# Nature40/pyradiotracking

Hardware: AMD Instinct MI355X
Metric: IQ MSamples/s analysed (STFT + detect + records), detected-signal parity vs CPU (higher is better)
Workload: dtype f32

## Files before the change

pyradiotracking_amd/csrc/rt_analyze.hip:

```cpp
#include <hip/hip_runtime.h>

#include <algorithm>
#include <cmath>
#include <cstdio>
#include <cstdlib>
#include <cstring>
#include <limits>
#include <new>
#include <string>
#include <type_traits>
#include <vector>

#include "rt_kernels.h"
#include "rt_general.h"
#include "rt_f64.h"
#include "rt_f64_sparse.h"
#include "rt_f64_rescue.h"
#include "rt_cells.h"
#include "rt_present.h"
#include "rt_chain.h"
#include "rt_record_iq.h"
#include "rt_record_stft.h"
#include "rt_record_stft_hop.h"
#include "rt_record_estimates.h"
// ... 219 lines not shown
struct InputStatsState {
    bool on = false;
    int max_chunks = 0;
    InputStatsSlot slot[kSlots];
};

}

struct rt_handle {
    rt_config cfg{};
    int R3 = 1, N = 256, LG = 16, GPW = 16;
    bool wcos = false;
    int big = 0;
    int QS = 0;
    int K = 1;
    int stride = 1;
    int L = 32;
    int max_seg = 0;
    std::vector<float> h_thr_s;
    int max_chunks = 0;
    bool two_level = false;
    int max_blocks = 0;
    hipStream_t s_scan = nullptr;
    bool own_scan_stream = false;
    hipStream_t s_detect = nullptr;
    std::string err;

    bool general = false;
    int log2n = 8;
    cf *d_twg = nullptr;
    bool bluestein = false;
    int gen_m = 0;
    cf *d_cwin = nullptr;
    cf *d_bfilt = nullptr;
    int n_cu = 256;
    uint32_t *d_work = nullptr;
    float *d_window = nullptr;
    float *d_window_t = nullptr;
    cf *d_tw1 = nullptr, *d_tw2 = nullptr;
    float *d_tail[kTails] = {nullptr, nullptr, nullptr};
    float *d_spec = nullptr;
    float *d_spec_part = nullptr;
    void *d_iq_stage[kSlots] = {nullptr, nullptr};
    size_t iq_stage_bytes[kSlots] = {0, 0};
    int64_t pool_want = 0;
    int64_t pool_max = 0;
    Slot slot[kSlots];

    int hot_cap = 8192, rec_cap = 1024, cand_cap = 32;
    bool group_detect = false;
    bool group_light = true;
    bool group_forced = false;
    size_t lds_large = 0, lds_small = 0, lds_dense = 0;

    bool lin = false;
    int32_t *d_sub_first = nullptr;
    std::vector<int32_t> h_sub_first;
    int32_t *h_sub_list = nullptr;
    int n_sub = 0;
    uint64_t sub_epoch = 0;
    float lin_c[3] = {0.f, 0.f, 0.f};

    AutoPolicy ap;
    int minsum_slot = -1;
    int run_cells = 1;
    uint64_t n_calls = 0;
    uint64_t test_enqueues = 0;
    int test_fail_lane = -1, test_fail_nth = 0;
    int tail_mode = 0;
    StreamLedger ledger;
    LedgerCall lc_saved;
    float *d_thr_s = nullptr, *d_cal_s = nullptr;
    StreamSettings *d_set_s = nullptr;
    std::vector<StreamSettings> h_set_s;

    rt_call_info info{};
    bool timing = false;

    std::vector<rt_handle *> kids;
    std::vector<int> kid_base;

    int rm_slot = -1;
    bool cells_full = false;
    int64_t cells_want = 0;

    size_t chunk_min_bytes = 0;
    const Slot *launch_mask = nullptr;
    std::vector<float> h_cal_s;

    F64State *f64 = nullptr;
    RecordIq *riq = nullptr;
    int iq_margin = -1;
    InputStatsState *ist = nullptr;
    std::vector<float> h_window;
};

namespace {

#define RT_HIP(h, expr)                                                                       \
    do {                                                                                      \
        hipError_t e_ = (expr);                                                               \
        if (e_ != hipSuccess) {                                                               \
            (h)->err = std::string(#expr) + ": " + hipGetErrorString(e_);                     \
            return RT_E_HIP;                                                                  \
        }                                                                                     \
    } while (0)

#ifdef RT_DIAG
extern "C" char **environ;
void warn_unknown_switches() {
    static bool done = false;
    if (done) return;
    done = true;
    static const char *const known[] = {"RT_EXP_ONE_LEVEL", "RT_EXP_TAIL", "RT_EXP_STREAMS", "RT_EXP_TAIL_PRIO", "RT_TEST_FAIL_LANE", "RT_STAMPS_DUMP"};
    for (char **e = environ; e && *e; ++e) {
        if (std::strncmp(*e, "RT_EXP_", 7) != 0 && std::strncmp(*e, "RT_TEST_", 8) != 0) continue;
        const char *eq = std::strchr(*e, '=');
        const std::string name(*e, eq ? (size_t)(eq - *e) : std::strlen(*e));
        bool ok = false;
        for (const char *k : known) ok = ok || name == k;
        if (!ok) std::fprintf(stderr, "librt_analyze_diag: environment variable %s is set but this build reads no such switch (known: RT_EXP_ONE_LEVEL, RT_EXP_TAIL, RT_EXP_STREAMS, RT_EXP_TAIL_PRIO, RT_TEST_FAIL_LANE, RT_STAMPS_DUMP)\n", name.c_str());
    }
}
#endif

#define RT_DEVICE_COPY(CHECK, dst, src, bytes)                     \
    do {                                                           \
        CHECK(hipMalloc(&dst, bytes));                             \
        CHECK(hipMemcpy(dst, src, bytes, hipMemcpyHostToDevice));  \
    } while (0)
#define RT_DEVICE_ZEROS(CHECK, dst, bytes) \
    do {                                   \
        CHECK(hipMalloc(&dst, bytes));     \
        CHECK(hipMemset(dst, 0, bytes));   \
    } while (0)

int fail_create(int code, const std::string &msg) {
    g_create_error = msg;
    return code;
}

size_t rec_lds_bytes(int rec_cap) { return (size_t)std::min(rec_cap, kDenseLdsRecords) * (8 + 8 + sizeof(rt_record)) + 16; }

void launch_detect_dense(rt_handle *h, int grid, hipStream_t st, const DetectArgs &a);

#define RT_SCAN_KERNEL(R3_, QS_) (stft_scan<R3_, MODEF, FMT == kFmtU8, LIN, QS_>)
#define RT_WG_KERNEL(B_, W_) (stft_wg<B_, MODEF, FMT == kFmtU8, W_>)
template <int MODE, int FMT, bool LIN>
void launch_stft_lin(rt_handle *h, const StftParams &p, int items, hipStream_t st) {
    constexpr int MODEF = MODE | (FMT == kFmtI16 ? kModeI16 : FMT == kFmtI8 ? kModeI8 : 0);
    if (h->big) {
        if constexpr (MODE <= 2) {
            if (h->big == 256) {
                if (h->wcos) hipLaunchKernelGGL(RT_WG_KERNEL(256, true), dim3(items), dim3(256), wg_lds_bytes(256), st, p);
                else hipLaunchKernelGGL(RT_WG_KERNEL(256, false), dim3(items), dim3(256), wg_lds_bytes(256), st, p);
            } else {
                if (h->wcos) hipLaunchKernelGGL(RT_WG_KERNEL(512, true), dim3(items), dim3(512), wg_lds_bytes(512), st, p);
                else hipLaunchKernelGGL(RT_WG_KERNEL(512, false), dim3(items), dim3(512), wg_lds_bytes(512), st, p);
            }
        }
        return;
    }
    if (scan_wave64(h->R3)) {
        const int wgs = std::min((items + kW64Waves - 1) / kW64Waves, h->n_cu);
        hipLaunchKernelGGL((stft_scan64<MODEF, FMT == kFmtU8, LIN>), dim3(wgs), dim3(kW64Block), 0, st, p);
        return;
    }
    const int blk = scan_block(h->R3);
    const int per_cu = scan_dma(h->R3, FMT, h->QS) ? 2 : std::min(((h->R3 <= RT_WG4_MAX_R3 || (FMT == kFmtU8 && h->R3 == 1)) ? 4 : 3) * (kBlock / blk), blk == 64 ? 12 : 4);
    const bool persist = scan_persistent(h->R3, MODE);
    const int blocks = persist ? std::min(items, h->n_cu * per_cu) : items;
    switch (h->QS ? -h->QS : h->R3) {
        case -8: hipLaunchKernelGGL(RT_SCAN_KERNEL(1, 8), dim3(blocks), dim3(blk), 0, st, p); break;
        case -4: hipLaunchKernelGGL(RT_SCAN_KERNEL(1, 4), dim3(blocks), dim3(blk), 0, st, p); break;
        case -2: hipLaunchKernelGGL(RT_SCAN_KERNEL(1, 2), dim3(blocks), dim3(blk), 0, st, p); break;
        case 1: hipLaunchKernelGGL(RT_SCAN_KERNEL(1, 0), dim3(blocks), dim3(blk), 0, st, p); break;
        case 2: hipLaunchKernelGGL(RT_SCAN_KERNEL(2, 0), dim3(blocks), dim3(blk), 0, st, p); break;
        case 4: hipLaunchKernelGGL(RT_SCAN_KERNEL(4, 0), dim3(blocks), dim3(blk), 0, st, p); break;
        case 8: hipLaunchKernelGGL(RT_SCAN_KERNEL(8, 0), dim3(blocks), dim3(blk), 0, st, p); break;
#if !RT_WAVE64_4096
        default: hipLaunchKernelGGL(RT_SCAN_KERNEL(16, 0), dim3(blocks), dim3(blk), 0, st, p); break;
#else
        default: break;
#endif
    }
}
#undef RT_SCAN_KERNEL
#undef RT_WG_KERNEL

template <int MODE, int FMT = kFmtC64>
void launch_stft(rt_handle *h, const StftParams &p, int blocks, hipStream_t st) {
    constexpr bool U8 = (FMT == kFmtU8);
    const Slot *const mk = (MODE != 3 && !p.stream_list) ? h->launch_mask : nullptr;
    if (mk) {
        const int S = h->cfg.n_streams;
        const int n_present = mk->lc.pc.n_present;
        if (n_present == 0) return;
        StftParams q = p;
        if (h->lin && !U8) {
            if (mk->n_lin_present > 0) {
                q.sub_first = nullptr;
                q.stream_list = mk->d_mask + (size_t)kMaskLinList * S;
                q.n_streams = mk->n_lin_present;
                q.spec_by_stream = 1;
                launch_stft_lin<MODE, FMT, (MODE != 3 && !U8)>(h, q, q.n_streams * p.blocks_per_stream, st);
            }
            if (mk->n_sub_present == 0) return;
            q = p;
            q.stream_list = mk->d_mask + (size_t)kMaskSubList * S;
            q.n_streams = mk->n_sub_present;
        } else {
            q.stream_list = mk->d_mask + (size_t)kMaskList * S;
            q.n_streams = n_present;
        }
        q.sub_first = nullptr;
        q.dc_flag = h->lin && !U8 ? nullptr : p.dc_flag;
        q.spec_by_stream = 1;
        launch_stft_lin<MODE, FMT, false>(h, q, q.n_streams * p.blocks_per_stream, st);
        return;
    }
    if (h->lin && MODE != 3 && !U8) {
        if (p.stream_list || h->n_sub == 0 || !p.sub_first) {
            StftParams q = p;
            if (p.stream_list) q.sub_first = nullptr;
            launch_stft_lin<MODE, FMT, (MODE != 3 && !U8)>(h, q, blocks, st);
        } else {
            launch_stft_lin<MODE, FMT, (MODE != 3 && !U8)>(h, p, blocks, st);
            StftParams q = p;
            q.sub_first = nullptr;
            q.dc_flag = nullptr;
            q.spec_by_stream = 1;
            q.stream_list = h->h_sub_list;
            q.n_streams = h->n_sub;
            launch_stft_lin<MODE, FMT, false>(h, q, h->n_sub * p.blocks_per_stream, st);
        }
    } else {
        launch_stft_lin<MODE, FMT, false>(h, p, blocks, st);
    }
}

void launch_general(rt_handle *h, const void *iq, int64_t stream_stride, int n_seg, float *spec, float *tail, int fmt, const int32_t *absent = nullptr) {
    if (h->bluestein) {
        BluesteinParams b{};
        b.absent = absent;
        b.iq = iq;
        b.stream_stride = stream_stride;
        b.n_streams = h->cfg.n_streams;
        b.n_seg = n_seg;
        b.nperseg = h->N;
        b.m = h->gen_m;
        b.log2m = h->log2n;
        b.tail_cols = h->K;
        b.cwin = h->d_cwin;
        b.bfilt = h->d_bfilt;
        b.tw = h->d_twg;
        b.spec = spec;
        b.tail = tail;
        const int blocks = h->cfg.n_streams * n_seg;
        const size_t lds = (size_t)h->gen_m * sizeof(cf);
#define RT_BLU(U_, B_)                                                                                                            \
    do {                                                                                                                          \
        if (fmt == kFmtU8) hipLaunchKernelGGL((stft_bluestein<kFmtU8, U_, B_>), dim3(blocks), dim3(B_), lds, h->s_scan, b);        \
        else if (fmt == kFmtI16) hipLaunchKernelGGL((stft_bluestein<kFmtI16, U_, B_>), dim3(blocks), dim3(B_), lds, h->s_scan, b); \
        else if (fmt == kFmtI8) hipLaunchKernelGGL((stft_bluestein<kFmtI8, U_, B_>), dim3(blocks), dim3(B_), lds, h->s_scan, b);   \
        else hipLaunchKernelGGL((stft_bluestein<kFmtC64, U_, B_>), dim3(blocks), dim3(B_), lds, h->s_scan, b);                     \
    } while (0)
        if (h->gen_m >= 16384) RT_BLU(4, 1024);
        else if (h->gen_m >= 8192) RT_BLU(4, 512);
        else if (h->gen_m >= 4096) RT_BLU(2, 512);
        else if (h->gen_m >= 2048) RT_BLU(2, 256);
        else RT_BLU(1, 256);
#undef RT_BLU
        return;
    }
    GeneralParams g{};
    g.absent = absent;
    g.iq = iq;
    g.stream_stride = stream_stride;
    g.n_streams = h->cfg.n_streams;
    g.n_seg = n_seg;
    g.nperseg = h->N;
    g.log2n = h->log2n;
    g.segs_per_block = std::min(64, std::max(1, 1024 / h->N));
    g.tail_cols = h->K;
    g.window = h->d_window;
    g.tw = h->d_twg;
    g.spec = spec;
    g.tail = tail;
    const int blocks = h->cfg.n_streams * ((n_seg + g.segs_per_block - 1) / g.segs_per_block);
    const size_t lds = (size_t)g.segs_per_block * h->N * sizeof(cf);
    if (fmt == kFmtU8) hipLaunchKernelGGL((stft_general<kFmtU8>), dim3(blocks), dim3(kGeneralBlock), lds, h->s_scan, g);
    else if (fmt == kFmtI16) hipLaunchKernelGGL((stft_general<kFmtI16>), dim3(blocks), dim3(kGeneralBlock), lds, h->s_scan, g);
    else if (fmt == kFmtI8) hipLaunchKernelGGL((stft_general<kFmtI8>), dim3(blocks), dim3(kGeneralBlock), lds, h->s_scan, g);
    else hipLaunchKernelGGL((stft_general<kFmtC64>), dim3(blocks), dim3(kGeneralBlock), lds, h->s_scan, g);
}

long long min_run_cells(const rt_handle *h) { return rt::min_run_cells(h->N, h->cfg.sample_rate, h->cfg.min_duration_s); }

int choose_chunk(const rt_config &cfg, const ScanFamily &fam, int n_streams, int n_seg) {
    return rt::choose_chunk(cfg.nperseg, fam.R3, fam.QS, scan_block(fam.R3), cfg.sample_rate, cfg.min_duration_s, cfg.segs_per_chunk, n_streams, n_seg);
}


StftParams make_stft_params(rt_handle *h, Slot &sl, const void *iq, int64_t stream_stride, int n_seg, int tail_write) {
    StftParams p{};
    p.iq = iq;
    p.stream_stride = stream_stride;
    p.n_streams = h->cfg.n_streams;
    p.n_seg = n_seg;
    p.segs_per_chunk = h->L;
    p.chunks = (n_seg + h->L - 1) / h->L;
// ... 4020 lines not shown
```

pyradiotracking_amd/csrc/rt_diag.h:

```cpp
#ifndef RT_DIAG_H
#define RT_DIAG_H

#ifdef RT_DIAG
#include <cstdlib>
#define RT_DIAG_ENV(name) std::getenv(name)
#else
#define RT_DIAG_ENV(name) (static_cast<const char *>(nullptr))
#if defined(RT_STAMPS) || defined(RT_ABLATE) || defined(RT_DETECT_ABLATE) || defined(RT_W64_ABL) || defined(RT_WG_ABL) || defined(RT_EXP_WG_HALF) || defined(RT_EXP_DMA1024) || defined(RT_EXP_WG_NOFENCE) || defined(RT_EXP_NOBAR0) || defined(RT_EXP_NOBAR1) || \
    defined(RT_EXP_ALIAS) || defined(RT_EXP_NOWIN) || defined(RT_EXP_PRIO) || defined(RT_ONE_WAVE_MAX_R3) || defined(RT_NO_PERSIST) ||                    \
    defined(RT_WG4_MAX_R3) || defined(RT_PK_R3_MASK) || defined(RT_BELOW_MAX_R3) || defined(RT_WAVE64_4096) || defined(RT_W64_PK) ||                       \
    defined(RT_W64_PREFETCH) || defined(RT_W64_Q2AHEAD) || defined(RT_EXP6) || defined(RT_EXP_U8_PK)
#error "laboratory switch (RT_STAMPS, RT_ABLATE, RT_EXP_*, RT_W64_*, RT_*_MAX_R3, ...) in a product build: add -DRT_DIAG (tools/variant.sh does)"
#endif
#endif

#endif
```

pyradiotracking_amd/csrc/rt_kernels.h:

```cpp
#ifndef RT_KERNELS_H
#define RT_KERNELS_H

#include <hip/hip_runtime.h>
#include <stdint.h>

#include <type_traits>

#include "../../include/rt_analyze.h"
#include "rt_diag.h"
#include "rt_core.h"
#include "rt_fft.h"

namespace rt {

constexpr int kBlock = 256;
constexpr int kRowF2 = 18;

struct StftParams {
    const void *iq;
    int64_t stream_stride;
    int32_t n_streams;
    int32_t n_seg;
    int32_t segs_per_chunk;
    int32_t chunks;
// ... 2638 lines not shown

template <class OnRun>
__device__ __forceinline__ bool scan_dense_row_blocked(const DetectParams &p, const float *row, int64_t stride,
                                                       double row_sum, int t_begin, int t_end, float *avg_out,
                                                       OnRun on_run) {
    const int T = p.n_seg;
    constexpr int B = 16;
    if (row_sum < 0.0) {
        double sum = 0.0;
        for (int t0 = 0; t0 < T; t0 += B) {
            float v[B];
#pragma unroll
            for (int k = 0; k < B; ++k) v[k] = (t0 + k < T) ? row[(int64_t)(t0 + k) * stride] : 0.f;
#pragma unroll
            for (int k = 0; k < B; ++k)
                if (t0 + k < T) sum += (double)v[k];
        }
        row_sum = sum;
    }
    const float avg = (float)row_sum / (float)T;
    *avg_out = avg;
    bool in_cont = (t_begin > 0) && cell_above(row[(int64_t)(t_begin - 1) * stride], avg, p.thr, p.snr);
    int b = -1;
    uint32_t prev = in_cont ? 1u : 0u;
    for (int t0 = t_begin; t0 < T; t0 += B) {
        float v[B];
#pragma unroll
        for (int k = 0; k < B; ++k) v[k] = (t0 + k < T) ? row[(int64_t)(t0 + k) * stride] : 0.f;
        const int nv = (T - t0 < B) ? (T - t0) : B;
        uint32_t m = 0;
#pragma unroll
        for (int k = 0; k < B; ++k) {
            const bool ab = !(v[k] < p.thr) & !(v[k] / avg < p.snr);
            m |= (ab ? 1u : 0u) << k;
        }
        const uint32_t valid = (1u << nv) - 1u;
        m &= valid;
        uint32_t tr = (m ^ ((m << 1) | prev)) & valid;
        prev = (m >> (nv - 1)) & 1u;
        const int kc = t_end - 1 - t0;
        int pos = 0;
        bool done = false;
        for (;;) {
            const int kt = tr ? __builtin_ctz(tr) : nv;
            const int chk = pos > kc ? pos : kc;
            if (b < 0 && chk < kt) {
                done = true;
                break;
            }
            if (kt >= nv) break;
            const int t = t0 + kt;
            if ((m >> kt) & 1u) {
                if (t < t_end) b = t;
            } else if (in_cont) {
                in_cont = false;
            } else if (b >= 0) {
                const int rb = b;
                b = -1;
                on_run(rb, t, avg);
            }
            tr &= tr - 1u;
            pos = kt + 1;
            if (kt >= kc && b < 0) {
                done = true;
                break;
            }
        }
        if (done) break;
    }
    return true;
}

template <bool GLOBAL>
__global__ __launch_bounds__(kDetBlock) void detect_dense(const DetectArgs a) {
    extern __shared__ __attribute__((aligned(16))) unsigned char smem[];
    const int s_pos = blockIdx.x;
    const int s = a.stream_list ? a.stream_list[s_pos] : s_pos;
    const int tid = threadIdx.x;
    const int F = a.n_bins;
    const int T = a.dp.n_seg;
    unsigned char *ptr = smem;
    RecLds l;
    if constexpr (GLOBAL) {
        l.rec = a.raw + (int64_t)s * a.rec_cap;
        l.ts_us = nullptr;
        l.dur_us = nullptr;
        l.count = a.raw_count + s;
    } else {
        l = carve_rec_lds(ptr, a.rec_cap);
        if (tid == 0) *l.count = 0;
    }
    __syncthreads();

    const DetectParams dp = stream_params(a, s);
    const float *sp = a.spec + (int64_t)s_pos * T * F;
    int Q = 1;
    if (a.psum)
        while (F * Q * 2 <= kDetBlock && Q * 2 * 64 <= T) Q *= 2;
    const int span = (T + Q - 1) / Q;
    const int n_items = (a.absent && a.absent[s] != 0) ? 0 : F * Q;
    for (int item = tid; item < n_items; item += kDetBlock) {
        const int fi = item % F, q = item / F;
        const int t_begin = q * span;
        const int t_end = (t_begin + span < T) ? t_begin + span : T;
        if (t_begin >= T) continue;
        const float *row = sp + fi;
        PrevCells prev{a.prev + ((int64_t)s * a.prev_cols + a.prev_cols) * F + fi, F};
        double row_sum = -1.0;
        if (a.psum) row_sum = row_sum_from_partials(a.psum + (int64_t)s * a.chunks * F + fi, a.chunks, F);
        float av = 0.f;
        auto on_run = [&](int b, int e, float avg) {
            int start;
            if (gate_run(dp, b, e, avg, prev, &start)) push_candidate(a, l, s, fi, start, e, avg, 0);
        };
        scan_dense_row_blocked(dp, row, F, row_sum, t_begin, t_end, &av, on_run);
    }
    int nrec;
    if constexpr (GLOBAL) {
        __threadfence();
        __syncthreads();
        nrec = __hip_atomic_load(l.count, __ATOMIC_RELAXED, __HIP_MEMORY_SCOPE_AGENT);
        if (nrec > a.rec_cap) nrec = a.rec_cap;
    } else {
        nrec = settled_count(a, l);
    }

    for (int c = tid >> 6; c < nrec; c += kDetBlock / 64) {
        rt_record &r = l.rec[c];
        const int start = r.start;
        const float *row = sp + r.fi;
        PrevCells prev{a.prev + ((int64_t)s * a.prev_cols + a.prev_cols) * F + r.fi, F};
        auto cell = [&](int k) -> float {
            const int t = start + k;
            return t < 0 ? prev(-t) : row[(int64_t)t * F];
        };
        const RunStats st = run_stats_wave(r.end - start, cell);
        if ((tid & 63) == 0) {
            r.max_p = st.max_p;
            r.mean_p = st.mean_p;
            r.std_db = st.std_db;
        }
    }
    if constexpr (!GLOBAL) {
        __syncthreads();
        publish_records(a, l, s, nrec);
        if (tid == 0) close_call(a);
    }
}

}

#include "rt_scan64.h"
#include "rt_scan_wg.h"
#endif
```

pyradiotracking_amd/csrc/rt_scan_wg.h:

```cpp
#ifndef RT_SCAN_WG_H
#define RT_SCAN_WG_H

namespace rt {

constexpr int kWgStage = 128;

#ifndef RT_WG_ABL
#define RT_WG_ABL 0
#endif
#ifndef RT_EXP_WG_HALF
#define RT_EXP_WG_HALF 0
#endif
__host__ __device__ constexpr bool wg_half(int blk) { return RT_EXP_WG_HALF != 0 && blk == 256; }
__host__ __device__ constexpr int wg_row(int blk) { return blk + 2; }
__host__ __device__ constexpr size_t wg_lds_bytes(int blk) { return sizeof(cf) * (wg_half(blk) ? 16 : 32) * (size_t)wg_row(blk); }
__host__ __device__ constexpr int wg_block(int nperseg) { return nperseg / 32; }

template <int BIT, int K, bool ONE>
__device__ __forceinline__ void wg_twiddle(cf (&v)[32], const cf (&wb)[5], cf f) {
    if constexpr (BIT < 0) {
        if constexpr (!ONE) v[K] = cmul(v[K], f);
    } else {
        wg_twiddle<BIT - 1, K, ONE>(v, wb, f);
        const cf g = ONE ? wb[BIT] : cmul(f, wb[BIT]);
        wg_twiddle<BIT - 1, K | (1 << BIT), false>(v, wb, g);
    }
}

template <int NP>
__device__ __forceinline__ void wg_emit(const StftParams &p, int s, int seg, const float (&Pp)[NP], uint32_t emit, int bin0, int bin_stride, uint2 *stg,
                                        int &stg_n, bool &gave_up) {
    if (gave_up || __builtin_amdgcn_ballot_w64(emit != 0) == 0) return;
    asm volatile("" : "+v"(bin0));
    const int lane = threadIdx.x & 63;
    const int cnt = __builtin_popcount(emit);
    int off = 0, need = 0;
    constexpr int PLANES = (NP == 32) ? 6 : 5;
#pragma unroll
    for (int k = 0; k < PLANES; ++k) {
        const unsigned long long m = __builtin_amdgcn_ballot_w64(((cnt >> k) & 1) != 0);
        off += (int)__builtin_amdgcn_mbcnt_hi((uint32_t)(m >> 32), __builtin_amdgcn_mbcnt_lo((uint32_t)m, 0)) << k;
        need += __builtin_popcountll(m) << k;
    }
    if (stg_n + need > kWgStage) {
        flush_stage(p, s, stg, stg_n);
        stg_n = 0;
    }
    if (need <= kWgStage) {
        uint32_t e = emit;
        int o = stg_n + off;
        while (__builtin_amdgcn_ballot_w64(e != 0u) != 0ull) {
            if (e) {
                const int q = __builtin_ctz(e);
                e &= e - 1u;
                const uint32_t key = ((uint32_t)(bin0 + bin_stride * q) << p.tbits) | (uint32_t)seg;
                stg[o++] = make_uint2(key, __float_as_uint(pick_range<0, NP>(Pp, q)));
            }
        }
        stg_n += need;
    } else {
        const uint32_t cnt16 = lane < kBuckets ? __hip_atomic_load(&p.hot_count[s * kBuckets + lane], __ATOMIC_RELAXED, __HIP_MEMORY_SCOPE_AGENT) : 0u;
        gave_up = __builtin_amdgcn_ballot_w64(cnt16 > (uint32_t)p.hot_cap) != 0;
#pragma unroll 1
        for (int q = 0; q < NP && !gave_up; ++q) {
            if (emit & (1u << q)) {
                const int bin = bin0 + bin_stride * q;
                const int bkt = bin & (kBuckets - 1);
                const uint32_t slot = atomicAdd(&p.hot_count[s * kBuckets + bkt], 1u);
                if (slot < (uint32_t)p.hot_cap)
                    p.hot[((int64_t)s * kBuckets + bkt) * p.hot_cap + slot] = make_uint2(((uint32_t)bin << p.tbits) | (uint32_t)seg, __float_as_uint(pick_range<0, NP>(Pp, q)));
            }
        }
    }
}

template <int BLK, int MODEF, bool U8, bool WCOS>
__global__ __launch_bounds__(BLK, wg_half(BLK) ? 3 : (BLK == 256 ? 2 : 1)) void stft_wg(const StftParams p) {
    constexpr int MODE = MODEF & (kModeI16 - 1);
    constexpr int FMT = scan_fmt(MODEF, U8);
    using raw_t = typename raw_of<FMT>::type;
    static_assert(BLK == 256 || BLK == 512, "nperseg 8192 / 16384");
    static_assert(MODE == 0 || MODE == 1 || MODE == 2, "sparse, dense, spectrogram only");
    constexpr int N = 32 * BLK, R = BLK / 16, S1 = wg_row(BLK), NW = BLK / 64;
    constexpr bool EMIT = (MODE == 0), SUMS = (MODE != 2), SPEC = (MODE == 1 || MODE == 2);
    constexpr bool HALF = wg_half(BLK);
    extern __shared__ __attribute__((aligned(16))) unsigned char wg_smem[];
    cf *const xs = reinterpret_cast<cf *>(wg_smem);
    __shared__ double red[2 * NW];
    __shared__ __attribute__((aligned(16))) cf tw2_lds[R * 16];
    __shared__ uint2 stage_lds[EMIT ? NW * kWgStage : 1];
    const int tid = threadIdx.x, lane = tid & 63;
    const int wave = __builtin_amdgcn_readfirstlane(tid >> 6);
    const int T = p.n_seg, L = p.segs_per_chunk;

    for (int idx = tid; idx < R * 16; idx += BLK) tw2_lds[idx] = p.tw2[idx];
    cf wb[5];
#pragma unroll
    for (int i = 0; i < 5; ++i) wb[i] = p.tw1[i * BLK + tid];

    const int item = blockIdx.x;
    const int s_pos = item % p.n_streams;
    const int s = p.stream_list ? p.stream_list[s_pos] : s_pos;
    const int cb = p.chunks - 1 - item / p.n_streams;
    const int c0 = cb * L;
    const raw_t *stream_iq = reinterpret_cast<const raw_t *>(p.iq) + (int64_t)s * p.stream_stride;
    const float thr = p.thr_s ? p.thr_s[s] : p.thr;

    float acc[32];
#pragma unroll
    for (int r = 0; r < 32; ++r) acc[r] = 0.f;
    constexpr int PAIRS = (R == 16) ? 2 : 1, NP = 32 / PAIRS;
    uint32_t next_hot[PAIRS];
#pragma unroll
    for (int e = 0; e < PAIRS; ++e) next_hot[e] = 0u;
    uint2 *const stg = stage_lds + (EMIT ? wave * kWgStage : 0);
    int stg_n = 0;
    bool gave_up = false;

    raw_t nxt[32];
    auto request_half = [&](int seg_req, int j0) {
        const int sg = __builtin_amdgcn_readfirstlane(seg_req);
        const raw_t *base = (RT_WG_ABL & 4) ? reinterpret_cast<const raw_t *>(p.iq) + (int64_t)(sg & 63) * N : stream_iq + (int64_t)(sg < 0 ? 0 : sg) * N;
        const rsrc_t r = make_rsrc(base, (sg >= 0 && sg < T) ? (uint32_t)(N * sizeof(raw_t)) : 0u);
#pragma unroll
        for (int j = 0; j < 16; ++j) nxt[j0 + j] = buf_load_iq(r, tid * (int)sizeof(raw_t), BLK * (j0 + j) * (int)sizeof(raw_t), raw_t{});
    };
    auto request = [&](int seg_req) {
        request_half(seg_req, 0);
        request_half(seg_req, 16);
    };
    float w[WCOS ? 1 : 32];
    const float wc0 = p.lin_c[0], wca = p.lin_c[1] * wb[0].x, wcb = p.lin_c[1] * wb[0].y;
    auto request_window = [&]() {
        if constexpr (WCOS) {
        } else if constexpr (RT_WG_ABL & 1) {
#pragma unroll
            for (int j = 0; j < 32; ++j) w[j] = 0.5f + 0.01f * j;
        } else {
            const rsrc_t rw = make_rsrc(p.window_t, (uint32_t)(N * sizeof(float)));
#pragma unroll
            for (int q = 0; q < 8; ++q) {
                const buf_f4 w4 = raw_buffer_load_f4(rw, tid * 128, q * 16, 0);
                w[4 * q] = w4.x;  w[4 * q + 1] = w4.y;  w[4 * q + 2] = w4.z;  w[4 * q + 3] = w4.w;
            }
        }
    };
    int n_steps = L;
    request(c0 + L - 1);
    request_window();
    __syncthreads();

    for (int i = 1; i <= n_steps; ++i) {
        const int seg = c0 + L - i;
        const bool halo = i > L;
        const bool active = seg < T && seg >= 0;
        cf v[32];
#pragma unroll
        for (int j = 0; j < 32; ++j) v[j] = to_cf(nxt[j]);
        if (!active) {
            if (i < n_steps) request(seg - 1);
            continue;
        }

        if constexpr (!(RT_WG_ABL & 2)) {
            cf s16[16], s8[8], s4[4];
#pragma unroll
            for (int j = 0; j < 16; ++j) s16[j] = cadd(v[j], v[j + 16]);
#pragma unroll
            for (int j = 0; j < 8; ++j) s8[j] = cadd(s16[j], s16[j + 8]);
#pragma unroll
// ... 74 lines not shown
#pragma unroll
                for (int kk = 0; kk < 8; ++kk) {
                    const float4 t = t2[kk];
                    if (kk) u[2 * kk] = cmul(u[2 * kk], cf{t.x, t.y});
                    u[2 * kk + 1] = cmul(u[2 * kk + 1], cf{t.z, t.w});
                }
#pragma unroll
                for (int pp = 0; pp < 16; ++pp) col[R * pp] = u[pp];
            }
            __syncthreads();
            __builtin_amdgcn_sched_barrier(0);
            const float4 *row = reinterpret_cast<const float4 *>(xs + (tid & 15) * S1 + R * (tid >> 4));
            cf u[16];
#pragma unroll
            for (int j = 0; j < 8; ++j) {
                const float4 q4 = row[j];
                u[2 * j] = cf{q4.x, q4.y};
                u[2 * j + 1] = cf{q4.z, q4.w};
            }
            if (h == 1 && i < n_steps) request_window();
            dft16(u);
            float Pp[16];
#pragma unroll
            for (int q = 0; q < 16; ++q) {
                const int r = 16 * h + q;
                Pp[q] = __builtin_fmaf(u[q].x, u[q].x, u[q].y * u[q].y);
                if constexpr (SUMS && !(RT_WG_ABL & 16)) {
                    if (!halo) acc[r] += Pp[q];
                }
                if constexpr (SPEC) raw_buffer_store_f1(Pp[q], rs_spec, bin_t * 4, (16 * h + 512 * q) * 4, 0);
                if constexpr (SUMS) {
                    if (to_tail) raw_buffer_store_f1(Pp[q], rs_tail, bin_t * 4, (16 * h + 512 * q) * 4, 0);
                }
            }
            if constexpr (EMIT && !(RT_WG_ABL & 8)) {
                float mxp = __builtin_fmaxf(Pp[0], Pp[1]);
#pragma unroll
                for (int q = 2; q < 16; ++q) mxp = __builtin_fmaxf(mxp, Pp[q]);
                uint32_t hot = 0;
                if (!(mxp < thr)) {
#pragma unroll
                    for (int q = 15; q >= 0; --q) hot = (hot << 1) | ((Pp[q] < thr) ? 0u : 1u);
                }
                const uint32_t emit = halo ? (next_hot[h] & ~hot) : (hot | next_hot[h]);
                wg_emit<16>(p, s, seg, Pp, emit, 16 * h + bin_t, 512, stg, stg_n, gave_up);
                next_hot[h] = hot;
                any_hot |= hot;
            }
        }
      } else {
#pragma unroll
        for (int k1 = 0; k1 < 32; ++k1) xs[k1 * S1 + tid] = v[k1];
        if constexpr (!WCOS) {
            __builtin_amdgcn_sched_barrier(0);
            if (i < n_steps) request(seg - 1);
            __builtin_amdgcn_sched_barrier(0);
        }
        __syncthreads();
        {
            const float4 *const t2 = reinterpret_cast<const float4 *>(tw2_lds + (tid % R) * 16);
#pragma unroll
            for (int e = 0; e < 2; ++e) {
#ifndef RT_EXP_WG_NOFENCE
                __builtin_amdgcn_sched_barrier(0);
#endif
                const int pi = tid + BLK * e;
                cf *const col = xs + (pi / R) * S1 + (pi % R);
                cf u[16];
#pragma unroll
                for (int c = 0; c < 16; ++c) u[c] = col[R * c];
                dft16(u);
#pragma unroll
                for (int kk = 0; kk < 8; ++kk) {
                    const float4 t = t2[kk];
                    if (kk) u[2 * kk] = cmul(u[2 * kk], cf{t.x, t.y});
                    u[2 * kk + 1] = cmul(u[2 * kk + 1], cf{t.z, t.w});
                }
#pragma unroll
                for (int pp = 0; pp < 16; ++pp) col[R * pp] = u[pp];
            }
        }
        __syncthreads();
#pragma unroll
        for (int e = 0; e < PAIRS; ++e) {
#ifndef RT_EXP_WG_NOFENCE
            __builtin_amdgcn_sched_barrier(0);
#endif
            const int ui = tid + BLK * e;
            const float4 *row = reinterpret_cast<const float4 *>(xs + (ui % 32) * S1 + R * (ui / 32));
            cf u[R];
#pragma unroll
            for (int j = 0; j < R / 2; ++j) {
                const float4 q4 = row[j];
                u[2 * j] = cf{q4.x, q4.y};
                u[2 * j + 1] = cf{q4.z, q4.w};
            }
            if (e == PAIRS - 1 && i < n_steps) request_window();
            if constexpr (R == 16) dft16(u); else dft32(u);
            float Pp[NP];
#pragma unroll
            for (int q = 0; q < NP; ++q) {
                const int r = e + PAIRS * q;
                Pp[q] = __builtin_fmaf(u[q].x, u[q].x, u[q].y * u[q].y);
                if constexpr (SUMS && !(RT_WG_ABL & 16)) {
                    if (!halo) acc[r] += Pp[q];
                }
                if constexpr (SPEC) raw_buffer_store_f1(Pp[q], rs_spec, tid * 4, BLK * r * 4, 0);
                if constexpr (SUMS) {
                    if (to_tail) raw_buffer_store_f1(Pp[q], rs_tail, tid * 4, BLK * r * 4, 0);
                }
            }
            if constexpr (EMIT && !(RT_WG_ABL & 8)) {
                float mxp = __builtin_fmaxf(Pp[0], Pp[1]);
#pragma unroll
                for (int q = 2; q < NP; ++q) mxp = __builtin_fmaxf(mxp, Pp[q]);
                uint32_t hot = 0;
                if (!(mxp < thr)) {
#pragma unroll
                    for (int q = NP - 1; q >= 0; --q) hot = (hot << 1) | ((Pp[q] < thr) ? 0u : 1u);
                }
                const uint32_t emit = halo ? (next_hot[e] & ~hot) : (hot | next_hot[e]);
                wg_emit<NP>(p, s, seg, Pp, emit, tid + BLK * e, BLK * PAIRS, stg, stg_n, gave_up);
                next_hot[e] = hot;
                any_hot |= hot;
            }
        }
      }
        if constexpr (EMIT && !(RT_WG_ABL & 8)) {
            if (i == L) {
                if (__syncthreads_or(c0 > 0 && any_hot != 0u)) {
                    n_steps = L + 1;
                    request(c0 - 1);
                    request_window();
                }
            }
        }
    }
    if constexpr (EMIT) {
        if (stg_n) flush_stage(p, s, stg, stg_n);
    }
    if constexpr (SUMS) {
        const rsrc_t rp = make_rsrc(p.psum + ((int64_t)s * p.blocks_per_stream + cb) * N, (uint32_t)(N * sizeof(float)));
        if constexpr (HALF) {
            const int bin_t = (tid & 15) + 32 * (tid >> 4);
#pragma unroll
            for (int r = 0; r < 32; ++r) raw_buffer_store_f1(acc[r], rp, bin_t * 4, (16 * (r / 16) + 512 * (r % 16)) * 4, 0);
        } else {
#pragma unroll
            for (int r = 0; r < 32; ++r) raw_buffer_store_f1(acc[r], rp, tid * 4, BLK * r * 4, 0);
        }
    }
}

}
#endif
```

Baseline: 784,900.

## Add 64-point-per-thread workgroup STFT kernel for large FFT sizes

Adds a new big-nperseg STFT kernel variant, enabled by default, in which each thread holds 64 complex points instead of 32. The workgroup is half as large and the FFT is factored as 64x64 plus a final radix-2 or radix-4 stage done across lanes with DPP butterflies. The LDS transpose is redesigned to use swizzled float4 reads and to move real and imaginary parts in two separate passes. Input is prefetched straight into LDS for the next segment. The aim is fewer LDS transposes and barriers per segment. The cost is higher register pressure: 64-entry arrays for the accumulators and FFT data, with occupancy bounded at 2 blocks.

```diff
diff --git a/pyradiotracking_amd/csrc/rt_analyze.hip b/pyradiotracking_amd/csrc/rt_analyze.hip
--- a/pyradiotracking_amd/csrc/rt_analyze.hip
+++ b/pyradiotracking_amd/csrc/rt_analyze.hip
@@ -395,11 +395,11 @@
     if (h->big) {
         if constexpr (MODE <= 2) {
             if (h->big == 256) {
-                if (h->wcos) hipLaunchKernelGGL(RT_WG_KERNEL(256, true), dim3(items), dim3(256), wg_lds_bytes(256), st, p);
-                else hipLaunchKernelGGL(RT_WG_KERNEL(256, false), dim3(items), dim3(256), wg_lds_bytes(256), st, p);
+                if (h->wcos) hipLaunchKernelGGL(RT_WG_KERNEL(256, true), dim3(items), dim3(wg_threads(256)), wg_lds_bytes(256), st, p);
+                else hipLaunchKernelGGL(RT_WG_KERNEL(256, false), dim3(items), dim3(wg_threads(256)), wg_lds_bytes(256), st, p);
             } else {
-                if (h->wcos) hipLaunchKernelGGL(RT_WG_KERNEL(512, true), dim3(items), dim3(512), wg_lds_bytes(512), st, p);
-                else hipLaunchKernelGGL(RT_WG_KERNEL(512, false), dim3(items), dim3(512), wg_lds_bytes(512), st, p);
+                if (h->wcos) hipLaunchKernelGGL(RT_WG_KERNEL(512, true), dim3(items), dim3(wg_threads(512)), wg_lds_bytes(512), st, p);
+                else hipLaunchKernelGGL(RT_WG_KERNEL(512, false), dim3(items), dim3(wg_threads(512)), wg_lds_bytes(512), st, p);
             }
         }
         return;
diff --git a/pyradiotracking_amd/csrc/rt_diag.h b/pyradiotracking_amd/csrc/rt_diag.h
--- a/pyradiotracking_amd/csrc/rt_diag.h
+++ b/pyradiotracking_amd/csrc/rt_diag.h
@@ -9,7 +9,7 @@
 #if defined(RT_STAMPS) || defined(RT_ABLATE) || defined(RT_DETECT_ABLATE) || defined(RT_W64_ABL) || defined(RT_WG_ABL) || defined(RT_EXP_WG_HALF) || defined(RT_EXP_DMA1024) || defined(RT_EXP_WG_NOFENCE) || defined(RT_EXP_NOBAR0) || defined(RT_EXP_NOBAR1) || \
     defined(RT_EXP_ALIAS) || defined(RT_EXP_NOWIN) || defined(RT_EXP_PRIO) || defined(RT_ONE_WAVE_MAX_R3) || defined(RT_NO_PERSIST) ||                    \
     defined(RT_WG4_MAX_R3) || defined(RT_PK_R3_MASK) || defined(RT_BELOW_MAX_R3) || defined(RT_WAVE64_4096) || defined(RT_W64_PK) ||                       \
-    defined(RT_W64_PREFETCH) || defined(RT_W64_Q2AHEAD) || defined(RT_EXP6) || defined(RT_EXP_U8_PK)
+    defined(RT_W64_PREFETCH) || defined(RT_W64_Q2AHEAD) || defined(RT_EXP6) || defined(RT_EXP_U8_PK) || defined(RT_WG64)
 #error "laboratory switch (RT_STAMPS, RT_ABLATE, RT_EXP_*, RT_W64_*, RT_*_MAX_R3, ...) in a product build: add -DRT_DIAG (tools/variant.sh does)"
 #endif
 #endif
diff --git a/pyradiotracking_amd/csrc/rt_kernels.h b/pyradiotracking_amd/csrc/rt_kernels.h
--- a/pyradiotracking_amd/csrc/rt_kernels.h
+++ b/pyradiotracking_amd/csrc/rt_kernels.h
@@ -2814,4 +2814,7 @@
 
 #include "rt_scan64.h"
 #include "rt_scan_wg.h"
+#if RT_WG64
+#include "rt_scan_wg64.h"
 #endif
+#endif
diff --git a/pyradiotracking_amd/csrc/rt_scan_wg.h b/pyradiotracking_amd/csrc/rt_scan_wg.h
--- a/pyradiotracking_amd/csrc/rt_scan_wg.h
+++ b/pyradiotracking_amd/csrc/rt_scan_wg.h
@@ -11,11 +11,18 @@
 #ifndef RT_EXP_WG_HALF
 #define RT_EXP_WG_HALF 0
 #endif
+#ifndef RT_WG64
+#define RT_WG64 1
+#endif
 __host__ __device__ constexpr bool wg_half(int blk) { return RT_EXP_WG_HALF != 0 && blk == 256; }
 __host__ __device__ constexpr int wg_row(int blk) { return blk + 2; }
-__host__ __device__ constexpr size_t wg_lds_bytes(int blk) { return sizeof(cf) * (wg_half(blk) ? 16 : 32) * (size_t)wg_row(blk); }
 __host__ __device__ constexpr int wg_block(int nperseg) { return nperseg / 32; }
-
+__host__ __device__ constexpr int wg_threads(int blk) { return RT_WG64 ? blk / 2 : blk; }
+__host__ __device__ constexpr size_t wg_lds_bytes(int blk) {
+    return RT_WG64 ? (size_t)(blk / 2) * 256 : sizeof(cf) * (wg_half(blk) ? 16 : 32) * (size_t)wg_row(blk);
+}
+
+#if !RT_WG64
 template <int BIT, int K, bool ONE>
 __device__ __forceinline__ void wg_twiddle(cf (&v)[32], const cf (&wb)[5], cf f) {
     if constexpr (BIT < 0) {
@@ -396,5 +403,7 @@
     }
 }
 
+#endif
+
 }
 #endif
diff --git a/pyradiotracking_amd/csrc/rt_scan_wg64.h b/pyradiotracking_amd/csrc/rt_scan_wg64.h
--- /dev/null
+++ b/pyradiotracking_amd/csrc/rt_scan_wg64.h
@@ -0,0 +1,363 @@
+#ifndef RT_SCAN_WG64_H
+#define RT_SCAN_WG64_H
+
+namespace rt {
+
+constexpr float kC256[128] = {1.0f, 0.99969881772995f, 0.9987954497337341f, 0.9972904324531555f, 0.9951847195625305f, 0.9924795627593994f, 0.9891765117645264f, 0.9852776527404785f, 0.9807852506637573f, 0.9757021069526672f, 0.9700312614440918f, 0.9637760519981384f, 0.9569403529167175f, 0.949528157711029f, 0.9415440559387207f, 0.9329928159713745f, 0.9238795042037964f, 0.91420978307724f, 0.903989315032959f, 0.89322429895401f, 0.8819212913513184f, 0.8700869679450989f, 0.8577286005020142f, 0.8448535799980164f, 0.8314695954322815f, 0.8175848126411438f, 0.803207516670227f, 0.7883464097976685f, 0.7730104327201843f, 0.7572088241577148f, 0.7409511208534241f, 0.7242470979690552f, 0.7071067690849304f, 0.6895405650138855f, 0.6715589761734009f, 0.6531728506088257f, 0.6343932747840881f, 0.6152315735816956f, 0.5956993103027344f, 0.5758081674575806f, 0.5555702447891235f, 0.5349976420402527f, 0.5141027569770813f, 0.49289819598197937f, 0.4713967442512512f, 0.4496113359928131f, 0.4275550842285156f, 0.40524131059646606f, 0.3826834261417389f, 0.3598950505256653f, 0.3368898630142212f, 0.3136817514896393f, 0.290284663438797f, 0.2667127549648285f, 0.24298018217086792f, 0.21910123527050018f, 0.19509032368659973f, 0.1709618866443634f, 0.1467304676771164f, 0.12241067737340927f, 0.0980171412229538f, 0.0735645666718483f, 0.049067676067352295f, 0.024541229009628296f, 0.0f, -0.024541229009628296f, -0.049067676067352295f, -0.0735645666718483f, -0.0980171412229538f, -0.12241067737340927f, -0.1467304676771164f, -0.1709618866443634f, -0.19509032368659973f, -0.21910123527050018f, -0.24298018217086792f, -0.2667127549648285f, -0.290284663438797f, -0.3136817514896393f, -0.3368898630142212f, -0.3598950505256653f, -0.3826834261417389f, -0.40524131059646606f, -0.4275550842285156f, -0.4496113359928131f, -0.4713967442512512f, -0.49289819598197937f, -0.5141027569770813f, -0.5349976420402527f, -0.5555702447891235f, -0.5758081674575806f, -0.5956993103027344f, -0.6152315735816956f, -0.6343932747840881f, -0.6531728506088257f, -0.6715589761734009f, -0.6895405650138855f, -0.7071067690849304f, -0.7242470979690552f, -0.7409511208534241f, -0.7572088241577148f, -0.7730104327201843f, -0.7883464097976685f, -0.803207516670227f, -0.8175848126411438f, -0.8314695954322815f, -0.8448535799980164f, -0.8577286005020142f, -0.8700869679450989f, -0.8819212913513184f, -0.89322429895401f, -0.903989315032959f, -0.91420978307724f, -0.9238795042037964f, -0.9329928159713745f, -0.9415440559387207f, -0.949528157711029f, -0.9569403529167175f, -0.9637760519981384f, -0.9700312614440918f, -0.9757021069526672f, -0.9807852506637573f, -0.9852776527404785f, -0.9891765117645264f, -0.9924795627593994f, -0.9951847195625305f, -0.9972904324531555f, -0.9987954497337341f, -0.99969881772995f};
+__device__ __forceinline__ constexpr float w256_re(int k) { return kC256[k]; }
+__device__ __forceinline__ constexpr float w256_im(int k) { return k < 64 ? kC256[k + 64] : -kC256[k - 64]; }
+
+__host__ __device__ constexpr int wg64_rot(int x, int sh) { return ((x << sh) | (x >> (4 - sh))) & 15; }
+
+template <int BIT, int K, bool ONE>
+__device__ __forceinline__ void wg64_twiddle(cf (&v)[64], const cf (&wb)[6], cf f) {
+    if constexpr (BIT < 0) {
+        if constexpr (!ONE) v[K] = cmul(v[K], f);
+    } else {
+        wg64_twiddle<BIT - 1, K, ONE>(v, wb, f);
+        const cf g = ONE ? wb[BIT] : cmul(f, wb[BIT]);
+        wg64_twiddle<BIT - 1, K | (1 << BIT), false>(v, wb, g);
+    }
+}
+
+template <int CTRL>
+__device__ __forceinline__ cf wg64_lane_bfly(cf a, float sgn) {
+    const float px = __int_as_float(__builtin_amdgcn_update_dpp(0, __float_as_int(a.x), CTRL, 0xF, 0xF, true));
+    const float py = __int_as_float(__builtin_amdgcn_update_dpp(0, __float_as_int(a.y), CTRL, 0xF, 0xF, true));
+    return cf{__builtin_fmaf(a.x, sgn, px), __builtin_fmaf(a.y, sgn, py)};
+}
+
+template <class raw_t, int B>
+__device__ __forceinline__ void wg64_prefetch(rsrc_t r, char *area, int lane, int wave) {
+    constexpr int SZ = sizeof(raw_t) == 2 ? 4 : 16;
+    constexpr int WP = 64 * (int)sizeof(raw_t);
+    constexpr int LP = WP / SZ;
+    constexpr int PARTS = 64 / LP;
+    constexpr int PB = B * (int)sizeof(raw_t);
+    const int k = lane / LP;
+    const int voff = (lane % LP) * SZ + (k & 1) * PB + (k >> 1) * 4 * PB + wave * WP;
+#pragma unroll
+    for (int j = 0; j < 32 / PARTS; ++j)
+        raw_buffer_load_lds(r, (__attribute__((address_space(3))) void *)(area + 64 * SZ * j), SZ, voff, 2 * PARTS * PB * j, 0, kAuxNT);
+}
+
+template <int BLK, int MODEF, bool U8, bool WCOS>
+__global__ __launch_bounds__(BLK / 2, 2) void stft_wg(const StftParams p) {
+    constexpr int MODE = MODEF & (kModeI16 - 1);
+    constexpr int FMT = scan_fmt(MODEF, U8);
+    using raw_t = typename raw_of<FMT>::type;
+    static_assert(BLK == 256 || BLK == 512, "nperseg 8192 / 16384");
+    static_assert(MODE == 0 || MODE == 1 || MODE == 2, "sparse, dense, spectrogram only");
+    constexpr int N = 32 * BLK, B = BLK / 2, W = B / 64, SH = (W == 2) ? 2 : 1;
+    constexpr bool EMIT = (MODE == 0), SUMS = (MODE != 2), SPEC = (MODE == 1 || MODE == 2);
+    extern __shared__ __attribute__((aligned(16))) unsigned char wg_smem[];
+    __shared__ double red[2 * W];
+    __shared__ uint2 stage_lds[EMIT ? W * kWgStage : 1];
+    const int tid = threadIdx.x, lane = tid & 63;
+    const int wave = __builtin_amdgcn_readfirstlane(tid >> 6);
+    const int T = p.n_seg, L = p.segs_per_chunk;
+    char *const area = reinterpret_cast<char *>(wg_smem) + wave * 16384;
+
+    const int item = blockIdx.x;
+    const int s_pos = item % p.n_streams;
+    const int s = p.stream_list ? p.stream_list[s_pos] : s_pos;
+    const int cb = p.chunks - 1 - item / p.n_streams;
+    const int c0 = cb * L;
+    const raw_t *stream_iq = reinterpret_cast<const raw_t *>(p.iq) + (int64_t)s * p.stream_stride;
+    const float thr = p.thr_s ? p.thr_s[s] : p.thr;
+
+    const int hx = tid % W;
+    const int bin0 = tid / W + 4096 * (W == 2 ? hx : (((hx & 1) << 1) | (hx >> 1)));
+    const cf w1 = p.tw1[tid];
+    const float wc0 = p.lin_c[0], wca = p.lin_c[1] * w1.x, wcb = p.lin_c[1] * w1.y;
+
+    float acc[64];
+#pragma unroll
+    for (int r = 0; r < 64; ++r) acc[r] = 0.f;
+    bits64 next_hot{0u, 0u};
+    uint2 *const stg = stage_lds + (EMIT ? wave * kWgStage : 0);
+    int stg_n = 0;
+    bool gave_up = false;
+
+    auto seg_rsrc = [&](int sg) {
+        return make_rsrc(stream_iq + (int64_t)(sg < 0 ? 0 : sg) * N, (sg >= 0 && sg < T) ? (uint32_t)(N * sizeof(raw_t)) : 0u);
+    };
+    const int seg_hi = __builtin_amdgcn_readfirstlane((c0 + L < T ? c0 + L : T) - 1);
+    const int len = seg_hi + 1 - c0;
+    int n_steps = len;
+    if (len > 0) wg64_prefetch<raw_t, B>(seg_rsrc(seg_hi), area, lane, wave);
+
+    for (int i = 1; i <= n_steps; ++i) {
+        const int seg = seg_hi + 1 - i;
+        const bool halo = i > len;
+        cf x[4][16];
+        {
+            const rsrc_t r = seg_rsrc(seg);
+            raw_t q2r[16], q3r[16];
+#pragma unroll
+            for (int j = 0; j < 16; ++j) q2r[j] = buf_load_iq(r, tid * (int)sizeof(raw_t), B * (2 + 4 * j) * (int)sizeof(raw_t), raw_t{});
+#pragma unroll
+            for (int j = 0; j < 16; ++j) q3r[j] = buf_load_iq(r, tid * (int)sizeof(raw_t), B * (3 + 4 * j) * (int)sizeof(raw_t), raw_t{});
+            __builtin_amdgcn_sched_barrier(0);
+            __builtin_amdgcn_s_waitcnt(0x8F70);
+            __builtin_amdgcn_sched_barrier(0);
+            int lane_a = lane;
+            asm volatile("" : "+v"(lane_a));
+            const raw_t *pre = reinterpret_cast<const raw_t *>(area);
+#pragma unroll
+            for (int j = 0; j < 16; ++j) {
+                x[0][j] = to_cf(pre[(2 * j) * 64 + lane_a]);
+                x[1][j] = to_cf(pre[(2 * j + 1) * 64 + lane_a]);
+            }
+#pragma unroll
+            for (int j = 0; j < 16; ++j) {
+                x[2][j] = to_cf(q2r[j]);
+                x[3][j] = to_cf(q3r[j]);
+            }
+        }
+        {
+            cf q[4];
+#pragma unroll
+            for (int n0 = 0; n0 < 4; ++n0) {
+                cf s8[8], s4[4];
+#pragma unroll
+                for (int j = 0; j < 8; ++j) s8[j] = cadd(x[n0][j], x[n0][j + 8]);
+#pragma unroll
+                for (int j = 0; j < 4; ++j) s4[j] = cadd(s8[j], s8[j + 4]);
+                q[n0] = cadd(cadd(s4[0], s4[2]), cadd(s4[1], s4[3]));
+            }
+            const cf sw = wave_sum<64>(cadd(cadd(q[0], q[2]), cadd(q[1], q[3])));
+            if (lane == 0) {
+                red[2 * wave] = (double)sw.x;
+                red[2 * wave + 1] = (double)sw.y;
+            }
+        }
+        __syncthreads();
+        cf v[64];
+        {
+            double tx = 0.0, ty = 0.0;
+#pragma unroll
+            for (int wv = 0; wv < W; ++wv) {
+                tx += red[2 * wv];
+                ty += red[2 * wv + 1];
+            }
+            const cf mean{(float)(tx / (double)N), (float)(ty / (double)N)};
+            float wca_ = wca, wcb_ = wcb;
+            asm volatile("" : "+v"(wca_), "+v"(wcb_));
+            int tid_w = tid;
+            asm volatile("" : "+v"(tid_w));
+#pragma unroll
+            for (int n0 = 0; n0 < 4; ++n0) {
+                cf a[16];
+                float wq4[WCOS ? 1 : 16];
+                if constexpr (!WCOS) {
+                    const rsrc_t rw = make_rsrc(p.window_t, (uint32_t)(N * sizeof(float)));
+#pragma unroll
+                    for (int j = 0; j < 16; ++j) wq4[j] = raw_buffer_load_f1(rw, (tid_w + (n0 & 1) * B) * 128, ((n0 >> 1) + 2 * j) * 4, 0);
+                }
+#pragma unroll
+                for (int j = 0; j < 16; ++j) {
+                    const int m = n0 + 4 * j;
+                    float wj;
+                    if constexpr (WCOS) {
+                        const float cbm = (m < 32) ? kW64Re[m] : -kW64Re[m - 32], msb = (m < 32) ? kW64Im[m] : -kW64Im[m - 32];
+                        wj = __builtin_fmaf(wca_, cbm, __builtin_fmaf(-wcb_, msb, wc0));
+                    } else {
+                        wj = wq4[j];
+                    }
+                    a[j] = cscale(csub(x[n0][j], mean), wj);
+                }
+                dft16(a);
+#pragma unroll
+                for (int j = 0; j < 16; ++j) v[n0 + 4 * j] = a[j];
+                __builtin_amdgcn_sched_barrier(0);
+            }
+        }
+        cf wq[6];
+        {
+            int tid_t = tid;
+            asm volatile("" : "+v"(tid_t));
+            const rsrc_t rt1 = make_rsrc(p.tw1, (uint32_t)(5 * BLK * sizeof(cf)));
+#pragma unroll
+            for (int i = 0; i < 5; ++i) {
+                const buf_f2 t = raw_buffer_load_f2(rt1, tid_t * 8, i * BLK * 8, 0);
+                wq[i] = cf{t.x, t.y};
+            }
+            const buf_f2 t = raw_buffer_load_f2(rt1, tid_t * 16, 4 * BLK * 8, 0);
+            wq[5] = cf{t.x, t.y};
+        }
+        __builtin_amdgcn_sched_barrier(0);
+        dft64_finish(v);
+        __builtin_amdgcn_sched_barrier(0);
+        wg64_twiddle<5, 0, true>(v, wq, cf{1.f, 0.f});
+        __builtin_amdgcn_sched_barrier(0);
+
+        cf u[64];
+        {
+            char *const ab = reinterpret_cast<char *>(wg_smem);
+            int tid_x = tid;
+            asm volatile("" : "+v"(tid_x));
+            const int h = tid_x % W, lp = tid_x / W;
+            const int st0 = h * 256 + ((4 * lp) ^ (wg64_rot(h, SH) << 4));
+            const int ld0 = tid_x * 256 + (wg64_rot(tid_x & 15, SH) << 4);
+            float re[64];
+#pragma unroll
+            for (int k1 = 0; k1 < 64; ++k1)
+                *reinterpret_cast<float *>(ab + W * k1 * 256 + (st0 ^ (wg64_rot((W * k1) & 15, SH) << 4))) = v[k1].x;
+            __syncthreads();
+#pragma unroll
+            for (int q = 0; q < 16; ++q) {
+                const float4 r4 = *reinterpret_cast<const float4 *>(ab + (ld0 ^ (q << 4)));
+                re[4 * q] = r4.x;  re[4 * q + 1] = r4.y;  re[4 * q + 2] = r4.z;  re[4 * q + 3] = r4.w;
+            }
+            __syncthreads();
+#pragma unroll
+            for (int k1 = 0; k1 < 64; ++k1)
+                *reinterpret_cast<float *>(ab + W * k1 * 256 + (st0 ^ (wg64_rot((W * k1) & 15, SH) << 4))) = v[k1].y;
+            __syncthreads();
+#pragma unroll
+            for (int q = 0; q < 16; ++q) {
+                const float4 r4 = *reinterpret_cast<const float4 *>(ab + (ld0 ^ (q << 4)));
+                u[4 * q] = cf{re[4 * q], r4.x};          u[4 * q + 1] = cf{re[4 * q + 1], r4.y};
+                u[4 * q + 2] = cf{re[4 * q + 2], r4.z};  u[4 * q + 3] = cf{re[4 * q + 3], r4.w};
+            }
+            wave_sync();
+        }
+        const int nxt = halo ? -1 : (seg > c0) ? seg - 1 : ((EMIT && c0 > 0) ? c0 - 1 : -1);
+        if (nxt >= 0) {
+            __builtin_amdgcn_s_waitcnt(0xC07F);
+            wg64_prefetch<raw_t, B>(seg_rsrc(nxt), area, lane, wave);
+        }
+        __builtin_amdgcn_sched_barrier(0);
+        dft64(u);
+        __builtin_amdgcn_sched_barrier(0);
+        {
+            int tid_r = tid;
+            asm volatile("" : "+v"(tid_r));
+            if constexpr (W == 2) {
+                const bool odd = (tid_r & 1) != 0;
+                const float sgn = odd ? -1.f : 1.f;
+#pragma unroll
+                for (int k = 0; k < 64; ++k) {
+                    if (k) {
+                        const cf m = cmul_const(u[k], w256_re(2 * k), w256_im(2 * k));
+                        u[k] = cf{odd ? m.x : u[k].x, odd ? m.y : u[k].y};
+                    }
+                    u[k] = wg64_lane_bfly<0xB1>(u[k], sgn);
+                }
+            } else {
+                const bool b0 = (tid_r & 1) != 0, b1 = (tid_r & 2) != 0;
+                const float sg0 = b0 ? -1.f : 1.f, sg1 = b1 ? -1.f : 1.f;
+#pragma unroll
+                for (int k = 0; k < 64; ++k) {
+                    if (k) {
+                        const cf m = cmul_const(u[k], w256_re(2 * k), w256_im(2 * k));
+                        u[k] = cf{b1 ? m.x : u[k].x, b1 ? m.y : u[k].y};
+                    }
+                    u[k] = wg64_lane_bfly<0x4E>(u[k], sg1);
+                    const cf m2 = k ? cmul_const(u[k], w256_re(k), w256_im(k)) : u[k];
+                    const cf m3{b1 ? m2.y : m2.x, b1 ? -m2.x : m2.y};
+                    u[k] = cf{b0 ? m3.x : u[k].x, b0 ? m3.y : u[k].y};
+                    u[k] = wg64_lane_bfly<0xB1>(u[k], sg0);
+                }
+            }
+        }
+        float P[64];
+#pragma unroll
+        for (int r = 0; r < 64; ++r) P[r] = __builtin_fmaf(u[r].x, u[r].x, u[r].y * u[r].y);
+        if constexpr (SUMS) {
+            if (!halo) {
+#pragma unroll
+                for (int r = 0; r < 64; ++r) acc[r] += P[r];
+            }
+        }
+        int bin_a = bin0;
+        asm volatile("" : "+v"(bin_a));
+        if constexpr (SPEC) {
+            const rsrc_t rs = make_rsrc(p.spec + ((int64_t)(p.spec_by_stream ? s : s_pos) * T + seg) * N, (uint32_t)(N * sizeof(float)));
+#pragma unroll
+            for (int r = 0; r < 64; ++r) raw_buffer_store_f1(P[r], rs, bin_a * 4, 256 * r, 0);
+        }
+        if constexpr (SUMS) {
+            const int tcol = seg - (T - p.tail_cols);
+            if (!halo && tcol >= 0) {
+                const rsrc_t rt_ = make_rsrc(p.tail + ((int64_t)s * p.tail_cols + tcol) * N, (uint32_t)(N * sizeof(float)));
+#pragma unroll
+                for (int r = 0; r < 64; ++r) raw_buffer_store_f1(P[r], rt_, bin_a * 4, 256 * r, 0);
+            }
+        }
+        if constexpr (EMIT) {
+            float mx = __builtin_fmaxf(__builtin_fmaxf(P[0], P[1]), P[2]);
+#pragma unroll
+            for (int r = 3; r < 63; r += 2) mx = __builtin_fmaxf(__builtin_fmaxf(mx, P[r]), P[r + 1]);
+            mx = __builtin_fmaxf(mx, P[63]);
+            bits64 hot{0u, 0u};
+            if (!(mx < thr)) {
+#pragma unroll
+                for (int r = 31; r >= 0; --r) {
+                    hot.lo = (hot.lo << 1) | ((P[r] < thr) ? 0u : 1u);
+                    hot.hi = (hot.hi << 1) | ((P[r + 32] < thr) ? 0u : 1u);
+                }
+            }
+            const bits64 emit = halo ? (next_hot & ~hot) : (hot | next_hot);
+            if (!gave_up && __builtin_amdgcn_ballot_w64(any(emit)) != 0ull) {
+                const uint32_t cnt = (uint32_t)(__builtin_popcount(emit.lo) + __builtin_popcount(emit.hi));
+                uint32_t before = 0;
+                int cells = 0;
+#pragma unroll
+                for (int b = 0; b < 7; ++b) {
+                    const unsigned long long m = __builtin_amdgcn_ballot_w64((cnt >> b) & 1u);
+                    before += (uint32_t)__builtin_amdgcn_mbcnt_hi((uint32_t)(m >> 32), __builtin_amdgcn_mbcnt_lo((uint32_t)m, 0)) << b;
+                    cells += __builtin_popcountll(m) << b;
+                }
+                if (stg_n + cells > kWgStage) {
+                    flush_stage(p, s, stg, stg_n);
+                    stg_n = 0;
+                }
+                const uint32_t key0 = ((uint32_t)bin_a << p.tbits) | (uint32_t)seg;
+                const bool staged = cells <= kWgStage;
+                if (!staged) {
+                    const uint32_t have = lane < kBuckets ? __hip_atomic_load(&p.hot_count[s * kBuckets + lane], __ATOMIC_RELAXED, __HIP_MEMORY_SCOPE_AGENT) : 0u;
+                    gave_up = __builtin_amdgcn_ballot_w64(have > (uint32_t)p.hot_cap) != 0ull;
+                }
+                if (!gave_up) {
+                    const int bkt = bin_a & (kBuckets - 1);
+                    uint32_t lo = emit.lo, hi = emit.hi;
+                    int idx = stg_n + (int)before;
+#pragma nounroll
+                    while ((lo | hi) != 0u) {
+                        int r;
+                        if (lo) { r = __builtin_ctz(lo); lo &= lo - 1u; } else { r = 32 + __builtin_ctz(hi); hi &= hi - 1u; }
+                        const uint2 cell = make_uint2(key0 + ((uint32_t)(64 * r) << p.tbits), __float_as_uint(pick64(P, r)));
+                        if (staged) {
+                            stg[idx++] = cell;
+                        } else {
+                            const uint32_t slot = atomicAdd(&p.hot_count[s * kBuckets + bkt], 1u);
+                            if (slot < (uint32_t)p.hot_cap) p.hot[((int64_t)s * kBuckets + bkt) * p.hot_cap + slot] = cell;
+                        }
+                    }
+                    if (staged) stg_n += cells;
+                }
+            }
+            next_hot = hot;
+        }
+
+        if constexpr (EMIT) {
+            if (i == len) {
+                if (__syncthreads_or(c0 > 0 && any(next_hot))) n_steps = len + 1;
+            }
+        }
+    }
+    __builtin_amdgcn_s_waitcnt(0x0F70);
+    if constexpr (EMIT) {
+        if (stg_n) flush_stage(p, s, stg, stg_n);
+    }
+    if constexpr (SUMS) {
+        const rsrc_t rp = make_rsrc(p.psum + ((int64_t)s * p.blocks_per_stream + cb) * N, (uint32_t)(N * sizeof(float)));
+#pragma unroll
+        for (int r = 0; r < 64; ++r) raw_buffer_store_f1(acc[r], rp, bin0 * 4, 256 * r, 0);
+    }
+}
+
+}
+#endif
```

Result: no change. 785,600 (median of 2 runs) (+0.1%).
